# robin-karlsson0/pc-accumulation-lib

Measured on AMD Instinct MI355X. Metric: Mpoints/s projected+accumulated and BEV frames/s @256x256; 1/2/4/8 GPU, higher is better.
Workload: dtype f64; 1 GPU; KITTI-360 single forward cam, 120k pts/frame, 200 m horizon (~201 live frames, 5169634 stored pts), one 256x256x21 BEV per integrated frame; points_per_frame=120000, bev_px=256, view_m=80

## Files before the change

pc-accumulation-lib_amd/csrc/pca_bev.hip:

```cpp
#include "pca_bev_common.h"
#include "pca_bev_view.h"
#include "pca_k1_body.h"
#include <cstdlib>
#include <mutex>

#define NFK (2 * TCELLS)
#ifndef AB_THREADS
#define AB_THREADS 1024
#endif
#define MAX_G 512
#ifndef BIN_RUNR
#define BIN_RUNR 4
#endif
#ifndef BIN_WPE
#define BIN_WPE 4
#endif
#ifndef BIN_UNR
#define BIN_UNR 4
#endif
#ifndef BIN_REG_P
#define BIN_REG_P 12
#endif
#ifndef C_THREADS
#define C_THREADS 256
// ... 70 lines not shown
    w.hi = (hi0 - w.lo > a.max_points) ? w.lo + a.max_points : hi0;
    const int G = a.G - a.Gk;
    const int64_t chunk = (w.hi - w.lo + G - 1) / G;
    g = (int)blockIdx.x;
    const int c = g - a.Gk;
    w.c_lo = w.lo + (int64_t)c * chunk;
    w.c_hi = w.c_lo + chunk < w.hi ? w.c_lo + chunk : w.hi;
    if (w.c_lo > w.hi) w.c_lo = w.c_hi = w.hi;
    return w;
}
__host__ __device__ __forceinline__ int64_t seg_stride(int64_t n, int G) { return (n + G - 1) / G; }
__device__ __forceinline__ bool bev_split(const BevArgs &a, int64_t window_points)
{
    return a.split == 2 || (a.split == 1 && window_points <= (int64_t)(a.G - a.Gk) * BIN_REG_P * AB_THREADS);
}

struct BinPoint { double x, y, z; uint32_t key; };
template <bool BAND>
__device__ __forceinline__ BinPoint bin_point(const BevArgs &a, const ViewConst &vc, const Window &w, const PendHi &pend_hi, int64_t p,
                                              double X, double Y, double Z, uint8_t D)
{
    BinPoint r;
    const bool moved = apply_owed(a.owed, pend_hi, p, X, Y, Z);
    if (moved && a.owed.write_back) { a.st.x[p] = X; a.st.y[p] = Y; a.st.z[p] = Z; }
    r.x = X; r.y = Y; r.z = Z;
    r.key = view_key_lean<BAND>(vc, X, Y, Z, D != 1, p >= w.sp ? 1u : 0u);
    return r;
}
template <bool I64>
__device__ __forceinline__ void bin_store(const BevArgs &a, const uint32_t *dynbits, uint32_t pos, uint32_t key, uint32_t rgbs, double z_store,
                                          double iv, float iv32)
{
    const pca_bev_params &q = a.prm;
    const unsigned sem = rgbs >> 24;
    uint32_t c = rgbs & 0xffffffu;
    if ((int)sem == q.road_class) c |= FLAG_ROAD;
    if ((dynbits[sem >> 5] >> (sem & 31u)) & 1u) c |= FLAG_DYNOBJ;
    const double z = z_store - q.origin[2];
    if (I64) {
        RecD r; r.z = z; r.inten = iv; r.c = c; r.fk = key & 127u;
        reinterpret_cast<RecD *>(a.recs)[pos] = r;
    } else {
        const float fi = iv32;
        if (fi < 0.0f) pca_raise(a.status, PCA_STATUS_NEGATIVE_INTENSITY);
        RecF r; r.z = z;
        r.iw = (__float_as_uint(fi) & 0x7fffffffu) | ((key & 1u) << 31);
        r.cw = c | (((key & 127u) >> 1) << 26);
        reinterpret_cast<RecF *>(a.recs)[pos] = r;
    }
}

__device__ unsigned long long g_dbg_stamps[1024][8];
#define BIN_STAMP(slot) do { if ((a.dbg & 32) && threadIdx.x == 0 && blockIdx.x < 1024) g_dbg_stamps[blockIdx.x][slot] = wall_clock64(); } while (0)
__device__ __forceinline__ void bin_scan_tables(const BevArgs &a, const uint32_t *s_h, uint32_t *s_cur, uint32_t *s_wsum, bool split, int g)
{
{
    const int per = (a.T + AB_THREADS - 1) / AB_THREADS;
    const int t0 = threadIdx.x * per;
    const int gp = bev_table_pos(a.Gp, g);
    uint32_t sum = 0;
    if (split) { for (int k = 0; k < per; ++k) sum += t0 + k < a.T ? s_h[2 * (t0 + k)] + s_h[2 * (t0 + k) + 1] : 0u; }
    else { for (int k = 0; k < per; ++k) sum += t0 + k < a.T ? s_h[t0 + k] : 0u; }
    const int lane = threadIdx.x & 63, wave = threadIdx.x >> 6;
    const uint32_t inc = wave_incl_scan_add(sum);
    if (lane == 63) s_wsum[wave] = inc;
    __syncthreads();
    uint32_t before = 0;
    for (int k = 0; k < wave; ++k) before += s_wsum[k];
    uint32_t run = before + inc - sum;
    for (int k = 0; k < per; ++k) {
        const int t = t0 + k;
        if (t >= a.T) break;
        if (split) {
            const uint32_t c0 = s_h[2 * t], c1 = s_h[2 * t + 1];
            s_cur[2 * t] = run;
            s_cur[2 * t + 1] = run + c0;
            a.bh[(int64_t)t * a.Gr + gp] = c0 + c1;
            a.boff[(int64_t)t * a.Gr + gp] = run;
            a.bh0[(int64_t)t * a.Gr + gp] = c0;
            run += c0 + c1;
        } else {
            const uint32_t c = s_h[t];
            s_cur[t] = run;
            a.bh[(int64_t)t * a.Gr + gp] = c;
            a.boff[(int64_t)t * a.Gr + gp] = run;
            run += c;
        }
    }
}
}

template <bool I64, bool BAND = false>
__device__ __forceinline__ void bev_tile_bin_body(const BevArgs &a)
{
    constexpr int REG_P = I64 ? 0 : BIN_REG_P;
    constexpr int UNR = BIN_RUNR;
    extern __shared__ uint32_t s_lds[];
    __shared__ uint32_t s_wsum[AB_THREADS / 64];
    __shared__ uint32_t s_dyn[8];
    uint32_t *s_h = s_lds;
    if (threadIdx.x < 8) {
        uint32_t w = (uint32_t)a.prm.dynobj_mask[0];
#pragma unroll
        for (int i = 1; i < 8; ++i) w = (int)threadIdx.x == i ? (uint32_t)(a.prm.dynobj_mask[i >> 1] >> (32 * (i & 1))) : w;
        s_dyn[threadIdx.x] = w;
    }
// ... 135 lines not shown
        const float *ib = a.st.intensity + w.c_lo;
#pragma unroll
        for (int j = 0; j < REG_P; ++j) {
            const uint32_t i = (uint32_t)j * AB_THREADS + threadIdx.x, ic = rkey[j] != KEY_INVALID ? i : 0u;
            rrgb[j] = cb[ic];
            rinten[j] = ib[ic];
        }
        {
            uint32_t touch = 0;
#pragma unroll
            for (int j = 0; j < REG_P; ++j) touch |= rrgb[j] ^ __float_as_uint(rinten[j]);
            asm volatile("" ::"v"(touch));
        }
#pragma unroll
        for (int j = 0; j < REG_P; ++j) {
            if (rkey[j] == KEY_INVALID) continue;
            const uint32_t pos = seg + atomicAdd(&s_cur[rkey[j] >> hs], 1u);
            bin_store<I64>(a, s_dyn, pos, rkey[j], rrgb[j], rz[j], 0.0, rinten[j]);
        }
    }
    BIN_STAMP(4);
    const bool stale = a.owed.n_pend > 0 && !a.owed.write_back;
    for (int64_t base = reg_hi + threadIdx.x; base < w.c_hi; base += MUNR * AB_THREADS) {
        uint32_t key[MUNR], pos[MUNR], rgbs[MUNR];
        double zz[MUNR], iv[MUNR], xs[MUNR], ys[MUNR];
#pragma unroll
        for (int u = 0; u < MUNR; ++u) {
            const int64_t p = base + u * AB_THREADS;
            key[u] = p < w.c_hi ? a.key[p - w.lo] : KEY_INVALID;
        }
#pragma unroll
        for (int u = 0; u < MUNR; ++u) {
            const int64_t p = base + u * AB_THREADS;
            const bool ok = key[u] != KEY_INVALID;
            rgbs[u] = ok ? a.st.rgbs[p] : 0u;
            zz[u] = ok ? a.st.z[p] : 0.0;
            xs[u] = (ok && stale) ? a.st.x[p] : 0.0;
            ys[u] = (ok && stale) ? a.st.y[p] : 0.0;
            if (I64) iv[u] = ok ? a.intensity64[p] : 0.0;
            else iv[u] = ok ? (double)a.st.intensity[p] : 0.0;
        }
#pragma unroll
        for (int u = 0; u < MUNR; ++u) {
            const int64_t p = base + u * AB_THREADS;
            const bool ok = key[u] != KEY_INVALID;
            if (ok && stale) apply_owed(a.owed, pend_hi, p, xs[u], ys[u], zz[u]);
            pos[u] = ok ? seg + atomicAdd(&s_cur[key[u] >> hs], 1u) : 0u;
        }
#pragma unroll
        for (int u = 0; u < MUNR; ++u)
            if (key[u] != KEY_INVALID) bin_store<I64>(a, s_dyn, pos[u], key[u], rgbs[u], zz[u], iv[u], (float)iv[u]);
    }
    BIN_STAMP(5);
    if ((a.dbg & 32) && threadIdx.x == 0 && blockIdx.x < 1024) { g_dbg_stamps[blockIdx.x][6] = (unsigned long long)a.owed.n_pend * 2 + a.owed.write_back; g_dbg_stamps[blockIdx.x][7] = __smid(); }
}

struct RecMap {
    uint32_t pre[1024 + 1];
    uint32_t base[1024];
    uint32_t wsum[16];
};
__device__ __forceinline__ uint32_t recmap_build(RecMap &M, const BevArgs &a, int tile, int nthreads, uint16_t *owner = nullptr, int half = -1)
{
    const int per = (a.Gr + nthreads - 1) / nthreads;
    const int g0 = threadIdx.x * per;
    const uint32_t *cnt = a.bh + (int64_t)tile * a.Gr, *off = a.boff + (int64_t)tile * a.Gr;
    uint32_t c[4] = {0, 0, 0, 0}, o[4] = {0, 0, 0, 0}, c0[4] = {0, 0, 0, 0}, sum = 0;
    int grp[4] = {0, 0, 0, 0};
#pragma unroll
    for (int k = 0; k < 4; ++k)
        if (k < per && g0 + k < a.Gr) {
            grp[k] = bev_table_group(a.Gp, g0 + k);
            if (grp[k] < a.G) {
                c[k] = cnt[g0 + k]; o[k] = off[g0 + k];
                if (half >= 0) c0[k] = a.bh0[(int64_t)tile * a.Gr + g0 + k];
            }
        }
    const int64_t lo = window_begin(a), hi0 = window_end(a);
    const int64_t n = hi0 - lo > a.max_points ? a.max_points : hi0 - lo;
    if (half >= 0 && bev_split(a, n)) {
#pragma unroll
        for (int k = 0; k < 4; ++k) { if (half == 0) c[k] = c0[k]; else { o[k] += c0[k]; c[k] -= c0[k]; } }
    }
    const uint32_t chunk = (uint32_t)seg_stride(n, a.G - a.Gk);
#pragma unroll
    for (int k = 0; k < 4; ++k)
        if (k < per && g0 + k < a.Gr) {
            M.base[g0 + k] = (grp[k] < a.Gk ? (uint32_t)grp[k] * K1_SEG : (uint32_t)a.Gk * K1_SEG + (uint32_t)(grp[k] - a.Gk) * chunk) + o[k];
            sum += c[k];
        }
    const int lane = threadIdx.x & 63, wave = threadIdx.x >> 6;
    const uint32_t inc = wave_incl_scan_add(sum);
    if (lane == 63) M.wsum[wave] = inc;
    __syncthreads();
    uint32_t run = inc - sum;
    for (int k = 0; k < wave; ++k) run += M.wsum[k];
#pragma unroll
    for (int k = 0; k < 4; ++k)
        if (k < per && g0 + k < a.Gr) {
            M.pre[g0 + k] = run;
            if (owner && run + c[k] <= RGB_CAP)
                for (uint32_t j = 0; j < c[k]; ++j) owner[run + j] = (uint16_t)(g0 + k);
            run += c[k];
        }
    if ((int)threadIdx.x == nthreads - 1) M.pre[a.Gr] = run;
    __syncthreads();
    return M.pre[a.Gr];
// ... 758 lines not shown
                uint4 w[UNR];
                const uint32_t at0 = walk.at;
#pragma unroll
                for (int u = 0; u < UNR; ++u) at[u] = r0 + u < r_hi ? recwalk_next(walk, L.M, a.Gr, r_hi) : at0;
#pragma unroll
                for (int u = 0; u < UNR; ++u) w[u] = recf_raw(a, at[u]);
#pragma unroll
                for (int u = 0; u < UNR; ++u) {
                    recf_fields(w[u], k[u], c[u], z[u], iv[u]);
                    if (!(r0 + u < r_hi)) { k[u] = RUN_NONE; c[u] = 0; }
                }
            }
#pragma unroll
            for (int u = 0; u < UNR; ++u) {
                if (k[u] == RUN_NONE || (!own && (int)(k[u] >> 1) / H_CELLS != half)) continue;
                if (k[u] != run.key) {
                    if (run.key != RUN_NONE) run_flush(L.S, extra, run);
                    run_reset(run, k[u]);
                }
                run_add(run, extra, c[u], z[u], iv[u], div255);
                uint32_t *row = hist + ((((k[u] >> 1) % H_CELLS) * 2 + (k[u] & 1u)) * 3) * 128;
#pragma unroll
                for (int ch = 0; ch < 3; ++ch) hist16_add(row + ch * 128, (c[u] >> (8 * ch)) & 255u, 1u);
            }
        }
        if (run.key != RUN_NONE) run_flush(L.S, extra, run);
        __syncthreads();
        if ((a.dbg & 8) && threadIdx.x == 0 && tile < 1024) g_dbg_stamps[tile][3 + 2 * half] = wall_clock64();
        for (int job = wave; job < H_CELLS * 3; job += H_THREADS / 64) {
            const int cl = job / 3, ch = job % 3, cell = half * H_CELLS + cl;
            const uint32_t n_p = L.S.cnt[2 * cell], n_f = L.S.cnt[2 * cell + 1];
            if (n_p > 0xffffu || n_f > 0xffffu) { if (lane == 0) L.overflow = 1; continue; }
            if (n_p + n_f == 0) continue;
            hist16_medians(L.S, hist + ((cl * 2 + 0) * 3 + ch) * 128, hist + ((cl * 2 + 1) * 3 + ch) * 128, cell, ch, n_p, n_f);
        }
        __syncthreads();
        if ((a.dbg & 8) && threadIdx.x == 0 && tile < 1024) g_dbg_stamps[tile][4 + 2 * half] = wall_clock64();
    }
    for (int cell = half * H_CELLS; L.overflow && cell < (half + 1) * H_CELLS; ++cell) {
        const uint32_t n_p = L.S.cnt[2 * cell], n_f = L.S.cnt[2 * cell + 1];
        if (n_p <= 0xffffu && n_f <= 0xffffu) continue;
        tile_cell_medians32<I64, H_THREADS>(L.S, L.hist, L.M, a, cell, r_lo, r_hi);
    }
    __syncthreads();
    tile_finalize_write<BAND>(a, L.S, reinterpret_cast<double(*)[TCELLS]>(smem), tile, H_THREADS, half * H_CELLS, (half + 1) * H_CELLS);
    __syncthreads();
    if ((a.dbg & 8) && threadIdx.x == 0 && tile < 1024) {
        g_dbg_stamps[tile][0] = t_begin; g_dbg_stamps[tile][1] = wall_clock64(); g_dbg_stamps[tile][2] = r_hi - r_lo;
        g_dbg_stamps[tile][7] = __smid();
    }
    }
}

struct BinK1Tail {
    const BevArgs &a;
    template <int PPT>
    __device__ __forceinline__ void operator()(const float4 (&p)[PPT], const uint32_t (&packed)[PPT], const uint64_t (&km)[PPT]) const
    {
        extern __shared__ uint32_t s_lds[];
        __shared__ uint32_t s_wsum[AB_THREADS / 64];
        __shared__ uint32_t s_dyn[8];
        const int64_t lo = window_begin(a), hi0 = window_end(a);
        const bool split = bev_split(a, hi0 - lo > a.max_points ? a.max_points : hi0 - lo);
        const int hs = split ? 6 : 7, n_hist = split ? 2 * a.T : a.T;
        uint32_t *s_h = s_lds, *s_cur = s_lds + n_hist;
        if (threadIdx.x < 8) {
            uint32_t w = (uint32_t)a.prm.dynobj_mask[0];
#pragma unroll
            for (int i = 1; i < 8; ++i) w = (int)threadIdx.x == i ? (uint32_t)(a.prm.dynobj_mask[i >> 1] >> (32 * (i & 1))) : w;
            s_dyn[threadIdx.x] = w;
        }
        for (int t = threadIdx.x; t < n_hist; t += AB_THREADS) s_h[t] = 0;
        __syncthreads();
        const ViewConst vc = view_const(a.prm, a.tx, a.band_r0, a.band_rows);
        const uint32_t set = a.k1_slot >= a.slot_split ? 1u : 0u;
        const int lane = threadIdx.x & 63;
        uint32_t rkey[PPT];
#pragma unroll
        for (int r = 0; r < PPT; ++r) {
            const bool kept = (km[r] >> lane) & 1ull;
            rkey[r] = view_key_lean(vc, (double)p[r].x, (double)p[r].y, (double)p[r].z, kept, set);
            if (rkey[r] != KEY_INVALID) atomicAdd(&s_h[rkey[r] >> hs], 1u);
        }
        __syncthreads();
        bin_scan_tables(a, s_h, s_cur, s_wsum, split, (int)blockIdx.x);
        __syncthreads();
        const uint32_t seg = (uint32_t)blockIdx.x * K1_SEG;
#pragma unroll
        for (int r = 0; r < PPT; ++r) {
            if (rkey[r] == KEY_INVALID) continue;
            const uint32_t pos = seg + atomicAdd(&s_cur[rkey[r] >> hs], 1u);
            bin_store<false>(a, s_dyn, pos, rkey[r], packed[r], (double)p[r].z, 0.0, p[r].w);
        }
    }
};
static_assert(K1_SEG == 1024 * 4, "a K1 piece holds one 1024 x 4 tile");
__global__ __launch_bounds__(AB_THREADS) __attribute__((amdgpu_waves_per_eu(BIN_WPE, BIN_WPE))) void bev_tile_bin_k1(const BevArgs a, const K1Args k)
{
    if ((int)blockIdx.x < a.Gk) k1_body<AB_THREADS, 4, false, false, false>(k, BinK1Tail{a});
    else bev_tile_bin_body<false>(a);
}

template <bool I64>
__global__ __launch_bounds__(AB_THREADS) __attribute__((amdgpu_waves_per_eu(BIN_WPE, BIN_WPE))) void bev_tile_bin(const BevArgs a) { bev_tile_bin_body<I64>(a); }
#if C_THREADS == 512
#define C_OCC __attribute__((amdgpu_waves_per_eu(6, 6)))
#else
#define C_OCC
#endif
template <bool I64>
__global__ __launch_bounds__(C_THREADS) C_OCC void bev_tile_cells(const BevArgs a) { bev_tile_cells_body<I64>(a); }
template <bool I64, bool EXTRA, bool OWN>
__global__ __launch_bounds__(H_THREADS) void bev_tile_cells_heavy(const BevArgs a) { bev_tile_cells_heavy_body<I64, EXTRA, OWN>(a); }
#define PCA_BEV_MANY_MAX 48
__constant__ BevArgs g_bev_many[PCA_BEV_MANY_MAX];
template <bool I64>
__global__ __launch_bounds__(AB_THREADS) __attribute__((amdgpu_waves_per_eu(BIN_WPE, BIN_WPE))) void bev_tile_bin_many()
{
    const BevArgs &a = g_bev_many[blockIdx.y];
    if ((int)blockIdx.x < a.G) bev_tile_bin_body<I64>(a);
}
template <bool I64>
__global__ __launch_bounds__(C_THREADS) C_OCC void bev_tile_cells_many()
{
    bev_tile_cells_body<I64>(g_bev_many[blockIdx.y]);
}
template <bool I64>
__global__ __launch_bounds__(H_THREADS) void bev_tile_cells_heavy_many()
{
    bev_tile_cells_heavy_body<I64, false, false>(g_bev_many[blockIdx.y]);
}
template <bool I64>
__global__ __launch_bounds__(AB_THREADS) __attribute__((amdgpu_waves_per_eu(BIN_WPE, BIN_WPE))) void bev_tile_bin_band(const BevArgs a) { bev_tile_bin_body<I64, true>(a); }
template <bool I64>
__global__ __launch_bounds__(C_THREADS) C_OCC void bev_tile_cells_band(const BevArgs a) { bev_tile_cells_body<I64, true>(a); }
template <bool I64, bool EXTRA>
__global__ __launch_bounds__(H_THREADS) void bev_tile_cells_heavy_band(const BevArgs a) { bev_tile_cells_heavy_body<I64, EXTRA, false, true>(a); }
template <bool I64>
__global__ __launch_bounds__(AB_THREADS) __attribute__((amdgpu_waves_per_eu(BIN_WPE, BIN_WPE))) void bev_tile_bin_band_many()
{
    const BevArgs &a = g_bev_many[blockIdx.y];
    if ((int)blockIdx.x < a.G) bev_tile_bin_body<I64, true>(a);
}
template <bool I64>
__global__ __launch_bounds__(C_THREADS) C_OCC void bev_tile_cells_band_many()
{
    bev_tile_cells_body<I64, true>(g_bev_many[blockIdx.y]);
}
template <bool I64>
__global__ __launch_bounds__(H_THREADS) void bev_tile_cells_heavy_band_many()
{
    bev_tile_cells_heavy_body<I64, false, false, true>(g_bev_many[blockIdx.y]);
}
// ... 217 lines not shown

static void bev_size_level1(pca_ctx *ctx, BevArgs &a, int nt, int one_round)
{
    if (nt == 0) { if (one_round > 0) { a.G = one_round; bev_table_order(a); } return; }
    const pca_ctx::K1Pending &pd = ctx->k1_pend;
    const int cap = max_groups(), G0 = a.G;
    if (one_round) one_round -= nt;
    a.G = one_round > 0 ? one_round + nt : (G0 + nt <= cap || (cap - 2 * nt) * 4 < 3 * G0) ? G0 + nt : cap - nt;
    a.Gk = nt; bev_table_order(a); a.k1_slot = pd.slot; a.k1_n = pd.fr.n;
    a.max_points = a.max_points - pd.fr.n;
}

static int bev_launch_raster(pca_ctx *ctx, const BevKernelSet &ks, const BevArgs &a, const K1Args *k1, size_t lds, hipStream_t s)
{
    if (k1) {
        PCA_LAUNCH_SHM(ctx, PCA_K_BEV_BIN, bev_tile_bin_k1, dim3(a.G), dim3(AB_THREADS), lds, s, a, *k1);
        pca_k1_pending_launched(ctx, s);
    } else PCA_LAUNCH_SHM(ctx, PCA_K_BEV_BIN, ks.bin, dim3(a.G), dim3(AB_THREADS), lds, s, a);
    PCA_LAUNCH(ctx, PCA_K_BEV_CELLS, ks.cells, dim3(a.T), dim3(C_THREADS), s, a);
    if (!a.heavy_launched) return 0;
    const int heavy_grid = a.T < ctx->n_cu ? a.T : ctx->n_cu;
    const BevKernel heavy = ks.heavy[a.extra != nullptr][a.split != 0];
    if (!heavy) { ctx->err = "bev: no heavy kernel for a split banded raster"; return -1; }
    PCA_LAUNCH_SHM(ctx, PCA_K_BEV_CELLS_HEAVY, heavy, dim3(heavy_grid), dim3(H_THREADS), HEAVY_LDS_BYTES, s, a);
    return 0;
}

int pca_bev_generate_chain(pca_ctx *ctx, const pca_store *store, const double *intensity64, const int64_t *frame_off,
                           int slot_begin, int slot_split, int slot_end, int64_t max_points, const pca_bev_params *prm,
                           const double *pending_Ts, const int *pending_slot_ends, int n_pending, int write_back,
                           void *workspace, int64_t workspace_bytes, double *planes, uint16_t *planes_f16,
                           double *extra_planes, void *stream)
{
    if (!ctx) return -1;
    const BevBinRange bin_range = {ctx->bin_valid, ctx->bin_first, ctx->bin_end};
    ctx->bin_valid = false;
    if (max_points < 1) max_points = 1;
    hipStream_t s = (hipStream_t)stream;
    PCA_CHECK(ctx, hipSetDevice(ctx->device));
    BevArgs a;
    if (bev_prepare(ctx, store, intensity64, frame_off, slot_begin, slot_split, slot_end, max_points, prm, pending_Ts,
                    pending_slot_ends, n_pending, write_back, workspace, workspace_bytes, planes, planes_f16, extra_planes, a))
        return -1;
    if (bev_set_lds_attributes(ctx)) return -1;
    const bool tuned = a.band_rows == a.tx;
    const BevKernelSet &ks = g_bev_kernels[intensity64 != nullptr][!tuned];
    K1Args k1a;
    int nt = 0;
    bev_decide_heavy(ctx, a, tuned);
    const size_t lds = bev_decide_split(a, tuned);
    if (bev_decide_k1_ride(ctx, a, tuned, lds, s, &k1a, &nt)) return -1;
    const int one_round = bev_decide_bin_range(ctx, a, tuned, bin_range);
    bev_size_level1(ctx, a, nt, one_round);
    ctx->last_level1[0] = a.G; ctx->last_level1[1] = a.Gk; ctx->last_level1[2] = a.bin_first; ctx->last_level1[3] = a.bin_end;
    if (ctx->profiling == 2) pca_prof_begin(ctx, PCA_K_BEV_UNIT, s);
    for (int r0 = 0, rows = a.band_rows; r0 < a.tx; r0 += rows) {
        if (!tuned) {
            bev_set_band(a, r0);
            if (r0 > 0 && a.owed.write_back) a.owed.n_pend = 0;
        }
        if (bev_launch_raster(ctx, ks, a, nt ? &k1a : nullptr, lds, s)) return -1;
    }
    if (ctx->profiling == 2) pca_prof_end(ctx, s);
    PCA_CHECK(ctx, hipGetLastError());
    return 0;
}

int pca_bev_generate_many(pca_ctx *ctx, const pca_store *store, const double *intensity64, const int64_t *frame_off,
                          const pca_bev_job *jobs, int n_jobs, int64_t max_points, void *workspace,
                          int64_t workspace_bytes, void *stream)
{
    if (!ctx) return -1;
    if (pca_k1_flush_pending(ctx)) return -1;
    ctx->bin_valid = false;
    if (!jobs || n_jobs < 1) { ctx->err = "bev: bad job list"; return -1; }
    if (n_jobs > 65535) { ctx->err = "bev: at most 65535 rasters per call"; return -1; }
    if (max_points < 1) max_points = 1;
    hipStream_t s = (hipStream_t)stream;
    PCA_CHECK(ctx, hipSetDevice(ctx->device));
    const int px = jobs[0].prm.px;
    PX_CHECK(ctx, px);
    const BevLayout l = bev_layout(max_points, px);
    const int64_t per = l.total;
    if (workspace_bytes < per * n_jobs + 256) { ctx->err = "bev: workspace too small for this many rasters"; return -1; }
    const int rows = band_rows(px), n_bands = (tiles_x(px) + rows - 1) / rows;
    const BevKernelSet &ks = g_bev_kernels[intensity64 != nullptr][n_bands > 1];
    const int64_t up_bytes = (int64_t)sizeof(BevArgs) * n_jobs * n_bands;
    if (ctx->bevm_busy) { PCA_CHECK(ctx, hipEventSynchronize(ctx->bevm_ev)); ctx->bevm_busy = false; }
    if (up_bytes > ctx->bevm_cap) {
        if (ctx->bevm_pin) PCA_CHECK(ctx, hipHostFree(ctx->bevm_pin));
        ctx->bevm_pin = nullptr; ctx->bevm_cap = 0;
        PCA_CHECK(ctx, hipHostMalloc(&ctx->bevm_pin, (size_t)(2 * up_bytes), hipHostMallocMapped));
        ctx->bevm_cap = 2 * up_bytes;
    }
    if (!ctx->bevm_ev) PCA_CHECK(ctx, hipEventCreateWithFlags(&ctx->bevm_ev, hipEventDisableTiming));
    BevArgs *ha = reinterpret_cast<BevArgs *>(ctx->bevm_pin);
    char *ws = reinterpret_cast<char *>(pca_align256(reinterpret_cast<intptr_t>(workspace)));
    for (int k = 0; k < n_jobs; ++k) {
        const pca_bev_job &j = jobs[k];
        if (j.prm.px != px) { ctx->err = "bev: the rasters of one call share the grid size"; return -1; }
        if (bev_prepare(ctx, store, intensity64, frame_off, j.slot_begin, j.slot_split, j.slot_end, max_points, &j.prm, nullptr,
                        nullptr, 0, 1, ws + per * k, per, j.planes, j.planes_f16, nullptr, ha[k]))
            return -1;
    }
    for (int b = n_bands - 1; b >= 0 && n_bands > 1; --b)
        for (int k = 0; k < n_jobs; ++k) {
// ... 26 lines not shown
    }
    PCA_CHECK(ctx, hipEventRecord(ctx->bevm_ev, s));
    ctx->bevm_busy = true;
    PCA_CHECK(ctx, hipEventRecord(last, s));
    if (ctx->profiling) pca_prof_end(ctx, s);
    PCA_CHECK(ctx, hipGetLastError());
    return 0;
}

struct WarpArgs {
    const uint16_t *in;
    uint16_t *out;
    int n_planes, px;
    double a1, a2, b1, b2;
};

__device__ __forceinline__ int warp_src(double c1, double c2, int k, int n)
{
    const double kd = (double)k;
    double v = rint(c1 * kd + c2 * (kd * kd));
    v = v < 0.0 ? 0.0 : (v > (double)(n - 1) ? (double)(n - 1) : v);
    return (int)v;
}

__global__ __launch_bounds__(256) void bev_warp(const WarpArgs a)
{
    const int iw = blockIdx.x * 256 + threadIdx.x, jw = blockIdx.y;
    if (iw >= a.px) return;
    const int i = warp_src(a.a1, a.a2, iw, a.px), j = warp_src(a.b1, a.b2, jw, a.px);
    const size_t plane = (size_t)a.px * a.px;
    for (int n = 0; n < a.n_planes; ++n) a.out[n * plane + (size_t)jw * a.px + iw] = a.in[n * plane + (size_t)j * a.px + i];
}

int pca_bev_warp(pca_ctx *ctx, const uint16_t *planes_f16, uint16_t *out_f16, int n_planes, int px, double a_1, double a_2,
                 double b_1, double b_2, void *stream)
{
    if (!ctx) return -1;
    if (!planes_f16 || !out_f16 || planes_f16 == out_f16 || n_planes < 1 || px < 1 || px > 65535) { ctx->err = "warp: bad arguments"; return -1; }
    if (!(a_1 == a_1 && a_2 == a_2 && b_1 == b_1 && b_2 == b_2)) { ctx->err = "warp: NaN coefficient"; return -1; }
    hipStream_t s = (hipStream_t)stream;
    PCA_CHECK(ctx, hipSetDevice(ctx->device));
    WarpArgs a;
    a.in = planes_f16; a.out = out_f16; a.n_planes = n_planes; a.px = px;
    a.a1 = a_1; a.a2 = a_2; a.b1 = b_1; a.b2 = b_2;
    hipLaunchKernelGGL(bev_warp, dim3((px + 255) / 256, px), dim3(256), 0, s, a);
    PCA_CHECK(ctx, hipGetLastError());
    return 0;
}

int pca_debug_bev_stamps(unsigned long long *out)
{
    return (int)hipMemcpyFromSymbol(out, HIP_SYMBOL(g_dbg_stamps), sizeof(unsigned long long) * 8192);
}

int pca_debug_bev_level1(const pca_ctx *ctx, int out[4])
{
    if (!ctx || !out) return -1;
    for (int k = 0; k < 4; ++k) out[k] = ctx->last_level1[k];
    return 0;
}

}
```

pc-accumulation-lib_amd/csrc/pca_k1_body.h:

```cpp
#pragma once
#include "pca_common.h"

__device__ __forceinline__ uint32_t k1_xcc_id() { return __builtin_amdgcn_s_getreg((3 << 11) | 20) & 7u; }
__device__ __forceinline__ int64_t k1_uniform_i64(int64_t v)
{
    const uint32_t lo = (uint32_t)__builtin_amdgcn_readfirstlane((int)(uint32_t)v);
    const uint32_t hi = (uint32_t)__builtin_amdgcn_readfirstlane((int)(uint32_t)((uint64_t)v >> 32));
    return (int64_t)(((uint64_t)hi << 32) | lo);
}
__device__ __forceinline__ uint32_t k1_mbcnt(uint64_t m)
{
    return __builtin_amdgcn_mbcnt_hi((uint32_t)(m >> 32), __builtin_amdgcn_mbcnt_lo((uint32_t)m, 0u));
}

#ifndef K1_STREAM_NT
#define K1_STREAM_NT 0
#endif
#ifndef K1_GATHER_MODE
#define K1_GATHER_MODE 0
#endif
template <typename T>
__device__ __forceinline__ T k1_gather(const T *p)
{
    typedef const __attribute__((address_space(1))) T *G;
// ... 103 lines not shown
                best[4 * i + 1] = (uint32_t)__builtin_amdgcn_readlane((int)w[i].y, c - 1);
                best[4 * i + 2] = (uint32_t)__builtin_amdgcn_readlane((int)w[i].z, c - 1);
                best[4 * i + 3] = (uint32_t)__builtin_amdgcn_readlane((int)w[i].w, c - 1);
            }
        }
        if (c < 64) break;
    }
    K1Frame fr;
    auto ptr = [&](int i) { return (uintptr_t)(((uint64_t)best[i + 1] << 32) | best[i]); };
    fr.pts = reinterpret_cast<const float *>(ptr(0));
    fr.rgb = reinterpret_cast<const uint8_t *>(ptr(2));
    fr.sem = reinterpret_cast<const uint8_t *>(ptr(4));
    fr.sem_gt = reinterpret_cast<const uint8_t *>(ptr(6));
    fr.n = (int32_t)best[8]; fr.tile0 = (int32_t)best[9]; fr.qpos0 = (int32_t)best[10]; fr.f = (int32_t)best[11];
    return fr;
}
static_assert(sizeof(K1Frame) == 48, "k1_find_frame reads a descriptor as three 16-byte words");

__device__ __forceinline__ K1Frame k1_frame_uniform(const K1Frame *f)
{
    typedef uint32_t u32x4 __attribute__((ext_vector_type(4)));
    const uint32_t lo = (uint32_t)__builtin_amdgcn_readfirstlane((int)(uint32_t)reinterpret_cast<uintptr_t>(f));
    const uint32_t hi = (uint32_t)__builtin_amdgcn_readfirstlane((int)(uint32_t)(reinterpret_cast<uintptr_t>(f) >> 32));
    const __attribute__((address_space(4))) u32x4 *p =
        reinterpret_cast<const __attribute__((address_space(4))) u32x4 *>(((uintptr_t)hi << 32) | lo);
    const u32x4 w0 = p[0], w1 = p[1], w2 = p[2];
    auto ptr = [](uint32_t a, uint32_t b) { return (uintptr_t)(((uint64_t)b << 32) | a); };
    K1Frame fr;
    fr.pts = reinterpret_cast<const float *>(ptr(w0.x, w0.y));
    fr.rgb = reinterpret_cast<const uint8_t *>(ptr(w0.z, w0.w));
    fr.sem = reinterpret_cast<const uint8_t *>(ptr(w1.x, w1.y));
    fr.sem_gt = reinterpret_cast<const uint8_t *>(ptr(w1.z, w1.w));
    fr.n = (int32_t)w2.x; fr.tile0 = (int32_t)w2.y; fr.qpos0 = (int32_t)w2.z; fr.f = (int32_t)w2.w;
    return fr;
}
template <int N>
__device__ __forceinline__ int k1_pick(const int (&v)[N], int q)
{
    int r = v[0];
#pragma unroll
    for (int i = 1; i < N; ++i) r = q == i ? v[i] : r;
    return r;
}

#define K1_INLINE_FRAMES 64
struct K1InlineFrames { K1Frame f[K1_INLINE_FRAMES]; };
static_assert(sizeof(K1Args) % alignof(K1InlineFrames) == 0, "inl follows a without padding");
__device__ __forceinline__ const K1Frame *k1_inline_frames()
{
    auto ka = __builtin_amdgcn_kernarg_segment_ptr();
    return reinterpret_cast<const K1Frame *>(reinterpret_cast<uintptr_t>(ka) + sizeof(K1Args));
}

struct K1NoTail { template <int PPT> __device__ __forceinline__ void operator()(const float4 (&)[PPT], const uint32_t (&)[PPT], const uint64_t (&)[PPT]) const {} };
template <int BLK, int PPT, bool SPLIT, bool BILIN, bool INL, typename Tail = K1NoTail>
__device__ __forceinline__ void k1_body(const K1Args &a, const Tail &tail = Tail())
{
    constexpr int TILE = BLK * PPT, NW = BLK / PCA_WAVE, NC = PPT * NW;
    static_assert(NC <= 64, "the per-(row, wave) counts are scanned by one wave");
    static_assert(TILE <= 65536, "tile-local indices are 16 bits");
    static_assert(PPT % 2 == 0, "phase 1 tests two rows per packed instruction");
    __shared__ float4 s_candp[TILE];
    __shared__ uint16_t s_cand[TILE];
    __shared__ uint32_t s_cnt[NC];
    __shared__ uint32_t s_filt[8];
    __shared__ long long s_excl;
    __shared__ uint32_t s_box[6];
    const int lane = threadIdx.x & 63;
    const int wave = __builtin_amdgcn_readfirstlane(threadIdx.x >> 6);
    K1_STAMP(0);

    K1Frame fr;
    int tin;
    if (!SPLIT) {
        fr = a.frames ? k1_find_frame<true>(a.frames, 0, a.n_frames, (int)blockIdx.x, lane) : a.one;
        tin = (int)blockIdx.x - fr.tile0;
    } else {
        const int q = blockIdx.x, f_lo = q * a.qbase + (q < a.qrem ? q : a.qrem), f_hi = f_lo + a.qbase + (q < a.qrem ? 1 : 0);
        if (a.tpf) {
            if (f_lo + (int)blockIdx.z >= f_hi) return;
            fr = INL ? k1_frame_uniform(k1_inline_frames() + f_lo + blockIdx.z)
                     : a.frames ? k1_frame_uniform(a.frames + f_lo + blockIdx.z) : a.one;
            tin = blockIdx.y;
        } else {
            if ((int)blockIdx.y >= k1_pick(a.qtiles, q)) return;
            fr = k1_find_frame<false>(a.frames, f_lo, f_hi, (int)blockIdx.y, lane);
            tin = (int)blockIdx.y - fr.qpos0;
        }
    }
    if (threadIdx.x < 8) {
        uint32_t w = (uint32_t)a.filt.w[0];
#pragma unroll
        for (int i = 1; i < 8; ++i) w = (int)threadIdx.x == i ? (uint32_t)(a.filt.w[i >> 1] >> (32 * (i & 1))) : w;
        s_filt[threadIdx.x] = w;
    }
    const int tile = fr.tile0 + tin;
    const int ftiles = fr.n > 0 ? (fr.n + TILE - 1) / TILE : 1;
    const int base_pt = tin * TILE;
    const int n_here = fr.n - base_pt < TILE ? fr.n - base_pt : TILE;
    const bool gt = fr.sem_gt != nullptr;
    const float *pts = fr.pts + 4 * (int64_t)base_pt;
    K1_STAMP(1);

    typedef float f2 __attribute__((ext_vector_type(2)));
    uint64_t cm[PPT];
    float4 v[PPT];
    if (n_here > 0) {
#pragma unroll
        for (int k = 0; k < PPT; ++k) {
            const int idx = k * BLK + (int)threadIdx.x;
            v[k] = k1_load_point(pts + 4 * (idx < n_here ? idx : n_here - 1), SPLIT);
        }
    } else {
#pragma unroll
        for (int k = 0; k < PPT; ++k) v[k] = make_float4(0.f, 0.f, 0.f, 0.f);
    }
    {
        const float *cu = a.cull;
        auto sp = [](float c) { f2 r; r.x = c; r.y = c; return r; };
#pragma unroll
        for (int k = 0; k < PPT; k += 2) {
            bool cand0 = k * BLK + (int)threadIdx.x < n_here, cand1 = (k + 1) * BLK + (int)threadIdx.x < n_here;
            if (!gt) {
                f2 x, y, z, m;
                x.x = v[k].x; x.y = v[k + 1].x; y.x = v[k].y; y.y = v[k + 1].y; z.x = v[k].z; z.y = v[k + 1].z;
                m.x = fmaxf(fmaxf(fabsf(x.x), fabsf(y.x)), fabsf(z.x));
                m.y = fmaxf(fmaxf(fabsf(x.y), fabsf(y.y)), fabsf(z.y));
                f2 M = __builtin_elementwise_fma(sp(cu[12]), m, sp(cu[13]));
                M.x = m.x > cu[16] ? __builtin_huge_valf() : M.x;
                M.y = m.y > cu[16] ? __builtin_huge_valf() : M.y;
                const f2 fx = __builtin_elementwise_fma(sp(cu[2]), z, __builtin_elementwise_fma(sp(cu[1]), y, __builtin_elementwise_fma(sp(cu[0]), x, sp(cu[3]))));
                const f2 fy = __builtin_elementwise_fma(sp(cu[6]), z, __builtin_elementwise_fma(sp(cu[5]), y, __builtin_elementwise_fma(sp(cu[4]), x, sp(cu[7]))));
                const f2 d = __builtin_elementwise_fma(sp(cu[10]), z, __builtin_elementwise_fma(sp(cu[9]), y, __builtin_elementwise_fma(sp(cu[8]), x, sp(cu[11]))));
                const f2 t1 = __builtin_elementwise_fma(sp(0.5f), d, fx), t2 = __builtin_elementwise_fma(sp(cu[14]), d, -fx);
                const f2 t3 = __builtin_elementwise_fma(sp(0.5f), d, fy), t4 = __builtin_elementwise_fma(sp(cu[15]), d, -fy);
                const int rej0 = (int)(d.x < -M.x) | (int)(t1.x < -M.x) | (int)(t2.x < -M.x) | (int)(t3.x < -M.x) | (int)(t4.x < -M.x);
                const int rej1 = (int)(d.y < -M.y) | (int)(t1.y < -M.y) | (int)(t2.y < -M.y) | (int)(t3.y < -M.y) | (int)(t4.y < -M.y);
                cand0 = cand0 && !rej0;
                cand1 = cand1 && !rej1;
            }
            cm[k] = __ballot(cand0);
            cm[k + 1] = __ballot(cand1);
            if (lane == 0) { s_cnt[k * NW + wave] = (uint32_t)__popcll(cm[k]); s_cnt[(k + 1) * NW + wave] = (uint32_t)__popcll(cm[k + 1]); }
        }
    }
    __syncthreads();
    K1_STAMP(2);
    uint32_t ncand;
    {
        const uint32_t c = lane < NC ? s_cnt[lane] : 0u;
        const uint32_t inc = wave_incl_scan_add(c);
        const uint32_t exc = inc - c;
        ncand = (uint32_t)__builtin_amdgcn_readlane((int)inc, NC - 1);
#pragma unroll
        for (int k = 0; k < PPT; ++k) {
            const uint32_t off = (uint32_t)__builtin_amdgcn_readlane((int)exc, k * NW + wave);
            if ((cm[k] >> lane) & 1ull) {
                const uint32_t o = off + k1_mbcnt(cm[k]);
                s_candp[o] = v[k];
                if (gt) s_cand[o] = (uint16_t)(k * BLK + threadIdx.x);
            }
        }
    }
    __syncthreads();
    K1_STAMP(3);

    uint64_t km[PPT];
    uint32_t packed[PPT];
    float4 p[PPT];
// ... 76 lines not shown
    K1_STAMP(4);
    uint32_t koff[PPT], total;
    {
        const uint32_t c = lane < NC ? s_cnt[lane] : 0u;
        const uint32_t inc = wave_incl_scan_add(c);
        const uint32_t exc = inc - c;
        total = (uint32_t)__builtin_amdgcn_readlane((int)inc, NC - 1);
#pragma unroll
        for (int r = 0; r < PPT; ++r) koff[r] = (uint32_t)__builtin_amdgcn_readlane((int)exc, r * NW + wave);
    }

    if (SPLIT) {
        float4 *rp = a.rec_p + (size_t)tile * TILE;
        uint32_t *rc = a.rec_c + (size_t)tile * TILE;
#pragma unroll
        for (int r = 0; r < PPT; ++r)
            if ((km[r] >> lane) & 1ull) {
                const uint32_t o = koff[r] + k1_mbcnt(km[r]);
#if K1_STREAM_NT & 2
                typedef float f4 __attribute__((ext_vector_type(4)));
                f4 w; w.x = p[r].x; w.y = p[r].y; w.z = p[r].z; w.w = p[r].w;
                __builtin_nontemporal_store(w, reinterpret_cast<__attribute__((address_space(1))) f4 *>(reinterpret_cast<uintptr_t>(rp + o)));
                __builtin_nontemporal_store(packed[r], reinterpret_cast<__attribute__((address_space(1))) uint32_t *>(reinterpret_cast<uintptr_t>(rc + o)));
#else
                rp[o] = p[r];
                rc[o] = packed[r];
#endif
            }
        if (threadIdx.x == 0) { a.counts[tile] = total; a.lastf[tile] = tin == ftiles - 1 ? fr.f : -1; }
        K1_STAMP(5);
        K1_STAMP(6);
        return;
    }

    if (a.st.frame_box) {
        uint32_t lo[3] = {0u, 0u, 0u}, hi[3] = {0u, 0u, 0u};
#pragma unroll
        for (int r = 0; r < PPT; ++r)
            if ((km[r] >> lane) & 1ull) {
                const float c[3] = {p[r].x, p[r].y, p[r].z};
#pragma unroll
                for (int k = 0; k < 3; ++k) {
                    const uint32_t o = pca_f32_ordered(c[k]);
                    hi[k] = hi[k] > o ? hi[k] : o;
                    lo[k] = lo[k] > ~o ? lo[k] : ~o;
                }
            }
#pragma unroll
        for (int k = 0; k < 3; ++k) {
            const uint32_t l = wave_reduce_max(lo[k]), h = wave_reduce_max(hi[k]);
            if (lane == 0 && h) { atomicMax(&s_box[2 * k], l); atomicMax(&s_box[2 * k + 1], h); }
        }
    }
    if (wave == 0) {
        const uint64_t e = lb_exclusive_prefix(a.state, tile, (uint64_t)total, a.epoch, a.status);
        if (lane == 0) s_excl = (long long)e;
    }
    __syncthreads();
    K1_STAMP(5);
    if (a.st.frame_box && threadIdx.x < 6 && s_box[threadIdx.x]) atomicMax(a.st.frame_box + (size_t)(a.first_slot + fr.f) * 6 + threadIdx.x, s_box[threadIdx.x]);
    const int64_t tile_base = a.frame_off[a.first_slot] + k1_uniform_i64(s_excl);
    const int64_t room64 = a.st.capacity - tile_base;
    const uint32_t room = room64 <= 0 ? 0u : (room64 > 0x7fffffffll ? 0x7fffffffu : (uint32_t)room64);
    double *xb = a.st.x + tile_base, *yb = a.st.y + tile_base, *zb = a.st.z + tile_base;
    float *ib = a.st.intensity + tile_base;
    uint32_t *cb = a.st.rgbs + tile_base;
    int32_t *nb = a.st.inst + tile_base;
    uint8_t *db = a.st.dyn + tile_base;
    bool overflow = false;
#pragma unroll
    for (int r = 0; r < PPT; ++r) {
        if (km[r] == 0) continue;
        if ((km[r] >> lane) & 1ull) {
            const uint32_t o = koff[r] + k1_mbcnt(km[r]);
            if (o >= room) { overflow = true; continue; }
            xb[o] = (double)p[r].x;
            yb[o] = (double)p[r].y;
            zb[o] = (double)p[r].z;
            ib[o] = p[r].w;
            cb[o] = packed[r];
            nb[o] = 0;
            db[o] = 0;
        }
    }
    if (overflow) pca_raise(a.status, PCA_STATUS_STORE_OVERFLOW);
    if (threadIdx.x == 0 && tin == ftiles - 1)
        a.frame_off[a.first_slot + fr.f + 1] = tile_base + total;
    K1_STAMP(6);
    tail.template operator()<PPT>(p, packed, km);
}
```

Baseline: 1555 Mpoints/s.

## Interleave BEV binning tail steps into K1 body around decoupled look-back wait

Splits the fused K1 tail into setup, key/histogram, scan and record phases and hooks them into the K1 body. Setup now runs before culling, keys and histogram are built after the tile aggregate is published, and the scan runs after the look-back walk. This lets tail work overlap the serial inter-block prefix wait instead of running after it. The look-back call is split into a separate publish and walk, the frame offset load is hoisted, and debug stamp buffers are added. The trade-off is more live registers and shared-state ordering across the new phase hooks.

Result: no change. 1567 Mpoints/s (median of 2 runs) (+0.8%).

```diff
diff --git a/pc-accumulation-lib_amd/csrc/pca_bev.hip b/pc-accumulation-lib_amd/csrc/pca_bev.hip
--- a/pc-accumulation-lib_amd/csrc/pca_bev.hip
+++ b/pc-accumulation-lib_amd/csrc/pca_bev.hip
@@ -146,6 +146,9 @@
 
 __device__ unsigned long long g_dbg_stamps[1024][8];
 #define BIN_STAMP(slot) do { if ((a.dbg & 32) && threadIdx.x == 0 && blockIdx.x < 1024) g_dbg_stamps[blockIdx.x][slot] = wall_clock64(); } while (0)
+__device__ unsigned long long g_dbg_stamps_hi[1024][8];
+#define RIDE_STAMP(slot) do { if ((a.dbg & 32) && threadIdx.x == 0 && blockIdx.x < 1024) g_dbg_stamps_hi[blockIdx.x][slot] = wall_clock64(); } while (0)
+#define RIDE_STAMP_LAST_WAVE() do { if ((a.dbg & 32) && (threadIdx.x & 63) == 0 && blockIdx.x < 1024) atomicMax(&g_dbg_stamps_hi[blockIdx.x][7], (unsigned long long)wall_clock64()); } while (0)
 __device__ __forceinline__ void bin_scan_tables(const BevArgs &a, const uint32_t *s_h, uint32_t *s_cur, uint32_t *s_wsum, bool split, int g)
 {
 {
@@ -387,7 +390,8 @@
             if (key[u] != KEY_INVALID) bin_store<I64>(a, s_dyn, pos[u], key[u], rgbs[u], zz[u], iv[u], (float)iv[u]);
     }
     BIN_STAMP(5);
-    if ((a.dbg & 32) && threadIdx.x == 0 && blockIdx.x < 1024) { g_dbg_stamps[blockIdx.x][6] = (unsigned long long)a.owed.n_pend * 2 + a.owed.write_back; g_dbg_stamps[blockIdx.x][7] = __smid(); }
+    if ((a.dbg & 32) && threadIdx.x == 0 && blockIdx.x < 1024) { g_dbg_stamps[blockIdx.x][6] = (unsigned long long)a.owed.n_pend * 2 + a.owed.write_back; g_dbg_stamps[blockIdx.x][7] = __smid(); g_dbg_stamps_hi[blockIdx.x][1] = 0; }
+    RIDE_STAMP(0);
 }
 
 struct RecMap {
@@ -1252,53 +1256,90 @@
     }
 }
 
+#ifndef K1_RIDE_EARLY
+#define K1_RIDE_EARLY 7
+#endif
+static_assert(K1_RIDE_EARLY == 0 || K1_RIDE_EARLY == 1 || K1_RIDE_EARLY == 3 || K1_RIDE_EARLY == 7, "each step needs the ones before it");
 struct BinK1Tail {
     const BevArgs &a;
-    template <int PPT>
-    __device__ __forceinline__ void operator()(const float4 (&p)[PPT], const uint32_t (&packed)[PPT], const uint64_t (&km)[PPT]) const
+    uint32_t *s_h, *s_cur;
+    bool split;
+    uint32_t rkey[4];
+    __device__ __forceinline__ int hs() const { return split ? 6 : 7; }
+    __device__ __forceinline__ uint32_t *wsum() const { __shared__ uint32_t s_wsum[AB_THREADS / 64]; return s_wsum; }
+    __device__ __forceinline__ uint32_t *dyn() const { __shared__ uint32_t s_dyn[8]; return s_dyn; }
+    __device__ __forceinline__ void setup()
     {
         extern __shared__ uint32_t s_lds[];
-        __shared__ uint32_t s_wsum[AB_THREADS / 64];
-        __shared__ uint32_t s_dyn[8];
         const int64_t lo = window_begin(a), hi0 = window_end(a);
-        const bool split = bev_split(a, hi0 - lo > a.max_points ? a.max_points : hi0 - lo);
-        const int hs = split ? 6 : 7, n_hist = split ? 2 * a.T : a.T;
-        uint32_t *s_h = s_lds, *s_cur = s_lds + n_hist;
+        split = bev_split(a, hi0 - lo > a.max_points ? a.max_points : hi0 - lo);
+        const int n_hist = split ? 2 * a.T : a.T;
+        s_h = s_lds; s_cur = s_lds + n_hist;
         if (threadIdx.x < 8) {
             uint32_t w = (uint32_t)a.prm.dynobj_mask[0];
 #pragma unroll
             for (int i = 1; i < 8; ++i) w = (int)threadIdx.x == i ? (uint32_t)(a.prm.dynobj_mask[i >> 1] >> (32 * (i & 1))) : w;
-            s_dyn[threadIdx.x] = w;
+            dyn()[threadIdx.x] = w;
         }
         for (int t = threadIdx.x; t < n_hist; t += AB_THREADS) s_h[t] = 0;
-        __syncthreads();
+        RIDE_STAMP(2);
+    }
+    template <int PPT>
+    __device__ __forceinline__ void keys(const float4 (&p)[PPT], const uint64_t (&km)[PPT])
+    {
+        static_assert(PPT == 4, "rkey holds one 1024 x 4 tile");
         const ViewConst vc = view_const(a.prm, a.tx, a.band_r0, a.band_rows);
         const uint32_t set = a.k1_slot >= a.slot_split ? 1u : 0u;
         const int lane = threadIdx.x & 63;
-        uint32_t rkey[PPT];
 #pragma unroll
         for (int r = 0; r < PPT; ++r) {
             const bool kept = (km[r] >> lane) & 1ull;
             rkey[r] = view_key_lean(vc, (double)p[r].x, (double)p[r].y, (double)p[r].z, kept, set);
-            if (rkey[r] != KEY_INVALID) atomicAdd(&s_h[rkey[r] >> hs], 1u);
-        }
+            if (rkey[r] != KEY_INVALID) atomicAdd(&s_h[rkey[r] >> hs()], 1u);
+        }
+        RIDE_STAMP(3);
+    }
+    __device__ __forceinline__ void scan()
+    {
+        bin_scan_tables(a, s_h, s_cur, wsum(), split, (int)blockIdx.x);
         __syncthreads();
-        bin_scan_tables(a, s_h, s_cur, s_wsum, split, (int)blockIdx.x);
-        __syncthreads();
+        RIDE_STAMP(4);
+    }
+    template <int PPT>
+    __device__ __forceinline__ void records(const float4 (&p)[PPT], const uint32_t (&packed)[PPT])
+    {
+        RIDE_STAMP(5);
         const uint32_t seg = (uint32_t)blockIdx.x * K1_SEG;
 #pragma unroll
         for (int r = 0; r < PPT; ++r) {
             if (rkey[r] == KEY_INVALID) continue;
-            const uint32_t pos = seg + atomicAdd(&s_cur[rkey[r] >> hs], 1u);
-            bin_store<false>(a, s_dyn, pos, rkey[r], packed[r], (double)p[r].z, 0.0, p[r].w);
-        }
+            const uint32_t pos = seg + atomicAdd(&s_cur[rkey[r] >> hs()], 1u);
+            bin_store<false>(a, dyn(), pos, rkey[r], packed[r], (double)p[r].z, 0.0, p[r].w);
+        }
+    }
+    __device__ __forceinline__ void front() { if (K1_RIDE_EARLY & 1) setup(); }
+    template <int PPT>
+    __device__ __forceinline__ void kept(const float4 (&p)[PPT], const uint64_t (&km)[PPT]) { if (K1_RIDE_EARLY & 2) keys<PPT>(p, km); }
+    __device__ __forceinline__ void placed() { if (K1_RIDE_EARLY & 4) scan(); }
+    template <int PPT>
+    __device__ __forceinline__ void done(const float4 (&p)[PPT], const uint32_t (&packed)[PPT], const uint64_t (&km)[PPT])
+    {
+        if (!(K1_RIDE_EARLY & 1)) { setup(); __syncthreads(); }
+        if (!(K1_RIDE_EARLY & 2)) { keys<PPT>(p, km); __syncthreads(); }
+        if (!(K1_RIDE_EARLY & 4)) scan();
+        records<PPT>(p, packed);
+        if ((a.dbg & 32) && threadIdx.x == 0 && blockIdx.x < 1024) {
+            g_dbg_stamps[blockIdx.x][7] = __smid(); g_dbg_stamps_hi[blockIdx.x][1] = 1; g_dbg_stamps_hi[blockIdx.x][6] = __smid();
+        }
+        RIDE_STAMP(0);
     }
 };
 static_assert(K1_SEG == 1024 * 4, "a K1 piece holds one 1024 x 4 tile");
 __global__ __launch_bounds__(AB_THREADS) __attribute__((amdgpu_waves_per_eu(BIN_WPE, BIN_WPE))) void bev_tile_bin_k1(const BevArgs a, const K1Args k)
 {
-    if ((int)blockIdx.x < a.Gk) k1_body<AB_THREADS, 4, false, false, false>(k, BinK1Tail{a});
+    if ((int)blockIdx.x < a.Gk) k1_body<AB_THREADS, 4, false, false, false>(k, BinK1Tail{a, nullptr, nullptr, false, {0u, 0u, 0u, 0u}});
     else bev_tile_bin_body<false>(a);
+    RIDE_STAMP_LAST_WAVE();
 }
 
 template <bool I64>
@@ -1622,6 +1663,11 @@
     if (bev_decide_k1_ride(ctx, a, tuned, lds, s, &k1a, &nt)) return -1;
     const int one_round = bev_decide_bin_range(ctx, a, tuned, bin_range);
     bev_size_level1(ctx, a, nt, one_round);
+    if (nt && (a.dbg & 32)) {
+        static void *stamps[64];
+        if (!stamps[ctx->device & 63]) PCA_CHECK(ctx, hipGetSymbolAddress(&stamps[ctx->device & 63], HIP_SYMBOL(g_dbg_stamps)));
+        k1a.dbg = reinterpret_cast<unsigned long long *>(stamps[ctx->device & 63]);
+    }
     ctx->last_level1[0] = a.G; ctx->last_level1[1] = a.Gk; ctx->last_level1[2] = a.bin_first; ctx->last_level1[3] = a.bin_end;
     if (ctx->profiling == 2) pca_prof_begin(ctx, PCA_K_BEV_UNIT, s);
     for (int r0 = 0, rows = a.band_rows; r0 < a.tx; r0 += rows) {
@@ -1754,6 +1800,10 @@
 {
     return (int)hipMemcpyFromSymbol(out, HIP_SYMBOL(g_dbg_stamps), sizeof(unsigned long long) * 8192);
 }
+int pca_debug_bev_stamps_hi(unsigned long long *out)
+{
+    return (int)hipMemcpyFromSymbol(out, HIP_SYMBOL(g_dbg_stamps_hi), sizeof(unsigned long long) * 8192);
+}
 
 int pca_debug_bev_level1(const pca_ctx *ctx, int out[4])
 {
diff --git a/pc-accumulation-lib_amd/csrc/pca_k1_body.h b/pc-accumulation-lib_amd/csrc/pca_k1_body.h
--- a/pc-accumulation-lib_amd/csrc/pca_k1_body.h
+++ b/pc-accumulation-lib_amd/csrc/pca_k1_body.h
@@ -179,9 +179,14 @@
     return reinterpret_cast<const K1Frame *>(reinterpret_cast<uintptr_t>(ka) + sizeof(K1Args));
 }
 
-struct K1NoTail { template <int PPT> __device__ __forceinline__ void operator()(const float4 (&)[PPT], const uint32_t (&)[PPT], const uint64_t (&)[PPT]) const {} };
+struct K1NoTail {
+    __device__ __forceinline__ void front() {}
+    template <int PPT> __device__ __forceinline__ void kept(const float4 (&)[PPT], const uint64_t (&)[PPT]) {}
+    __device__ __forceinline__ void placed() {}
+    template <int PPT> __device__ __forceinline__ void done(const float4 (&)[PPT], const uint32_t (&)[PPT], const uint64_t (&)[PPT]) {}
+};
 template <int BLK, int PPT, bool SPLIT, bool BILIN, bool INL, typename Tail = K1NoTail>
-__device__ __forceinline__ void k1_body(const K1Args &a, const Tail &tail = Tail())
+__device__ __forceinline__ void k1_body(const K1Args &a, Tail tail = Tail())
 {
     constexpr int TILE = BLK * PPT, NW = BLK / PCA_WAVE, NC = PPT * NW;
     static_assert(NC <= 64, "the per-(row, wave) counts are scanned by one wave");
@@ -242,6 +247,8 @@
 #pragma unroll
         for (int k = 0; k < PPT; ++k) v[k] = make_float4(0.f, 0.f, 0.f, 0.f);
     }
+    const int64_t first_off = SPLIT ? 0 : a.frame_off[a.first_slot];
+    tail.front();
     {
         const float *cu = a.cull;
         auto sp = [](float c) { f2 r; r.x = c; r.y = c; return r; };
@@ -424,14 +431,17 @@
             if (lane == 0 && h) { atomicMax(&s_box[2 * k], l); atomicMax(&s_box[2 * k + 1], h); }
         }
     }
+    if (wave == 0 && lane == 0) lb_publish_aggregate(a.state, tile, (uint64_t)total, a.epoch);
+    tail.template kept<PPT>(p, km);
     if (wave == 0) {
-        const uint64_t e = lb_exclusive_prefix(a.state, tile, (uint64_t)total, a.epoch, a.status);
+        const uint64_t e = lb_walk(a.state, tile, (uint64_t)total, a.epoch, a.status);
         if (lane == 0) s_excl = (long long)e;
     }
     __syncthreads();
     K1_STAMP(5);
+    tail.placed();
     if (a.st.frame_box && threadIdx.x < 6 && s_box[threadIdx.x]) atomicMax(a.st.frame_box + (size_t)(a.first_slot + fr.f) * 6 + threadIdx.x, s_box[threadIdx.x]);
-    const int64_t tile_base = a.frame_off[a.first_slot] + k1_uniform_i64(s_excl);
+    const int64_t tile_base = first_off + k1_uniform_i64(s_excl);
     const int64_t room64 = a.st.capacity - tile_base;
     const uint32_t room = room64 <= 0 ? 0u : (room64 > 0x7fffffffll ? 0x7fffffffu : (uint32_t)room64);
     double *xb = a.st.x + tile_base, *yb = a.st.y + tile_base, *zb = a.st.z + tile_base;
@@ -459,5 +469,5 @@
     if (threadIdx.x == 0 && tin == ftiles - 1)
         a.frame_off[a.first_slot + fr.f + 1] = tile_base + total;
     K1_STAMP(6);
-    tail.template operator()<PPT>(p, packed, km);
-}
+    tail.template done<PPT>(p, packed, km);
+}
```
